# ATTron/astroz

Hardware: AMD Instinct MI355X
Metric: propagations/sec, 13,478 sats x 1,440 times, at 1/2/4/8 MI355X (higher is better)
Workload: dtype f64

## Files before the change

astroz_amd/csrc/astroz_hip.hip:

```cpp
#include "../../include/astroz_hip.h"

#include <hip/hip_runtime.h>
#include <dlfcn.h>
#include <rccl/rccl.h>

#include <algorithm>
#include <atomic>
#include <cmath>
#include <condition_variable>
#include <deque>
#include <map>
#include <cstdio>
#include <cstdlib>
#include <cstring>
#include <mutex>
#include <new>
#include <memory>
#include <string>
#include <thread>
#include <type_traits>
#include <vector>

#include "kernels.h"
#include "passes_kernel.h"
// ... 729 lines not shown
    if (c->d_times.ensure(n_times) != AZ_OK) return AZ_ERR_HIP;
    HIP_TRY(hipMemcpyAsync(c->d_times.p, times, sizeof(double) * n_times, hipMemcpyHostToDevice, st));
    c->have_offsets = offsets != nullptr;
    if (offsets) {
        if (c->d_offsets.ensure(c->n) != AZ_OK) return AZ_ERR_HIP;
        HIP_TRY(hipMemcpyAsync(c->d_offsets.p, offsets, sizeof(double) * c->n, hipMemcpyHostToDevice, st));
    }
    c->have_mask = mask != nullptr;
    if (mask) {
        if (c->d_mask.ensure(c->n) != AZ_OK) return AZ_ERR_HIP;
        HIP_TRY(hipMemcpyAsync(c->d_mask.p, mask, c->n, hipMemcpyHostToDevice, st));
    }
    if (mode != AZ_OUT_TEME) {
        if (c->d_sin.ensure(n_times) != AZ_OK || c->d_cos.ensure(n_times) != AZ_OK) return AZ_ERR_HIP;
        hipLaunchKernelGGL(k_gmst, dim3((unsigned)((n_times + 255) / 256)), dim3(256), 0, st, c->d_times.p,
                           (unsigned)n_times, reference_jd, c->d_sin.p, c->d_cos.p);
        HIP_TRY(hipGetLastError());
    }
    c->cached_n_times = (unsigned)n_times;
    c->cached_mode = mode;
    c->seeds_valid = false;
    drop_graphs(c);
    for (auto &pl : c->plan) pl.valid = false;
    c->last_plan = -1;
    c->uniform_step = 0.0;
    c->delta_max = 0.0;
    c->delta_wide = false;
    c->grid_t0 = n_times ? times[0] : 0.0;
    if (n_times >= 2) {
        double t0 = times[0], step = (times[n_times - 1] - t0) / (double)(n_times - 1);
        double tmax = std::max(std::fabs(t0), std::fabs(times[n_times - 1]));
        const double tol = 4.0 * 2.220446049250313e-16 * std::max(tmax, std::fabs(step));
        bool uni = std::isfinite(step) && step != 0.0;
        double dmax = 0.0;
        for (size_t i = 1; uni && i < n_times; ++i) {
            dmax = std::max(dmax, std::fabs(times[i] - std::fma((double)i, step, t0)));
            uni = dmax <= AZ_DELTA_MAX;
        }
        if (uni && dmax > tol) {
            c->h_delta.assign(n_times + AZ_DELTA_SEG, 0.0f);
            for (size_t i = 0; i < n_times; ++i) c->h_delta[i] = (float)(times[i] - std::fma((double)i, step, t0));
            if (c->d_delta.ensure(c->h_delta.size()) != AZ_OK) return AZ_ERR_HIP;
            HIP_TRY(hipMemcpyAsync(c->d_delta.p, c->h_delta.data(), sizeof(float) * c->h_delta.size(), hipMemcpyHostToDevice, st));
            c->h_delta64.assign(n_times + AZ_DELTA_SEG, 0.0);
            for (size_t i = 0; i < n_times; ++i) c->h_delta64[i] = times[i] - std::fma((double)i, step, t0);
            if (c->d_delta64.ensure(c->h_delta64.size()) != AZ_OK) return AZ_ERR_HIP;
            HIP_TRY(hipMemcpyAsync(c->d_delta64.p, c->h_delta64.data(), sizeof(double) * c->h_delta64.size(), hipMemcpyHostToDevice, st));
            c->delta_max = dmax * (1.0 + 1e-6) + 1e-12;
        }
        if (!uni && n_times >= 64) {
            const double nn = (double)n_times, im = 0.5 * (nn - 1.0);
            double tm = 0.0;
            for (size_t i = 0; i < n_times; ++i) tm += times[i];
            tm /= nn;
            double sxy = 0.0, sxx = 0.0;
            for (size_t i = 0; i < n_times; ++i) {
                sxy += ((double)i - im) * (times[i] - tm);
                sxx += ((double)i - im) * ((double)i - im);
            }
            step = sxy / sxx;
            t0 = tm - step * im;
            bool ok = std::isfinite(step) && std::isfinite(t0) && step != 0.0;
            dmax = 0.0;
            for (size_t i = 0; ok && i < n_times; ++i) {
                dmax = std::max(dmax, std::fabs(times[i] - std::fma((double)i, step, t0)));
                ok = dmax <= AZ_DELTA_WIDE_MAX;
            }
            if (ok && dmax <= 0.5 * std::fabs(step)) {
                c->h_delta64.assign(n_times + AZ_DELTA_SEG, 0.0);
                for (size_t i = 0; i < n_times; ++i) c->h_delta64[i] = times[i] - std::fma((double)i, step, t0);
                if (c->d_delta64.ensure(c->h_delta64.size()) != AZ_OK) return AZ_ERR_HIP;
                HIP_TRY(hipMemcpyAsync(c->d_delta64.p, c->h_delta64.data(), sizeof(double) * c->h_delta64.size(), hipMemcpyHostToDevice, st));
                c->delta_max = dmax * (1.0 + 1e-6) + 1e-12;
                c->delta_wide = true;
                c->grid_t0 = t0;
                uni = true;
            }
        }
        if (uni) {
            if (c->d_inc.ensure((size_t)2 * AZ_INC_NUM * c->n_pad) != AZ_OK) return AZ_ERR_HIP;
            hipLaunchKernelGGL(k_prep_inc, dim3((unsigned)((c->n + 255) / 256)), dim3(256), 0, st, c->d_el.p, c->n, c->n_pad,
                               step, c->d_inc.p);
            HIP_TRY(hipGetLastError());
            if (c->d_fast_rec.ensure((size_t)FR_NUM * c->n_pad) != AZ_OK) return AZ_ERR_HIP;
            hipLaunchKernelGGL(k_prep_rec, dim3((unsigned)((c->n + 255) / 256)), dim3(256), 0, st, c->d_el.p, c->d_flags.p, c->n, c->n_pad,
                               c->d_inc.p, c->d_fast_rec.p);
            HIP_TRY(hipGetLastError());
            c->uniform_step = step;
        }
    }
    try {
        c->h_times.assign(times, times + n_times);
        if (offsets) c->h_offsets.assign(offsets, offsets + c->n);
        if (mask) c->h_mask.assign(mask, mask + c->n);
        c->staged_ref_jd = reference_jd;
        c->staged_stream = st;
        c->staged_valid = true;
    } catch (const std::bad_alloc &) {
        c->staged_valid = false;
    }
    return AZ_OK;
}

int32_t prepare_deep(azh_constellation *c, PropArgs &d, hipStream_t st, bool rows, bool beside_bulk = false)
{
    const unsigned n_times = d.n_times;
    d.list = c->d_list.p + (rows ? c->off_deep_cat : c->n_sgp4);
    d.n_list = c->n_sdp4;
    d.tile = auto_tile(c->n_sdp4, n_times, c->tile_sdp4, 8);
    d.tile_forced = c->tile_sdp4 ? c->tile_sdp4 : (rows && beside_bulk && c->n_sgp4 >= 4u * c->n_sdp4 ? rows_tile(c->n_sgp4, n_times, c->tile_sgp4) : 0u);
    const unsigned seed_tile = rows ? 64u : d.tile;
    const unsigned n_tiles = (n_times + seed_tile - 1) / seed_tile;
    if (!c->seeds_valid || c->seeds_tile != seed_tile || c->seeds_rows != rows) {
        if (c->capturing) return AZ_RC_EAGER;
        drop_graphs(c);
        if (c->d_seeds.ensure((size_t)n_tiles * 3 * c->n_sdp4) != AZ_OK) return AZ_ERR_HIP;
        if (c->d_node_cache.p == nullptr) {
            if (c->d_node_cache.ensure(3 * c->n_pad) != AZ_OK) return AZ_ERR_HIP;
            HIP_TRY(hipMemsetAsync(c->d_node_cache.p, 0, sizeof(double) * 3 * c->n_pad, st));
        }
        hipLaunchKernelGGL(k_deep_seed, dim3((c->n_sdp4 + 63) / 64), dim3(64), 0, st, c->d_el.p, c->d_flags.p, c->n_pad,
                           d.list, c->n_sdp4, d.times, n_times, d.offsets, seed_tile, c->d_seeds.p, rows ? 1 : 0, c->d_node_cache.p);
        HIP_TRY(hipGetLastError());
        c->seeds_valid = true;
        c->seeds_tile = seed_tile;
        c->seeds_rows = rows;
    }
    d.seeds = c->d_seeds.p;
    return AZ_OK;
}

int32_t ensure_plan(azh_constellation *c, PropArgs &a, const FastShape &shape, hipStream_t st)
{
    azh_constellation::FastPlan &pl = c->plan[shape.kind];
    const unsigned n_list = a.n_list;
    const unsigned n_seg = (a.n_times + std::min(shape.tile_c, shape.tile_e) - 1) / std::min(shape.tile_c, shape.tile_e);
    if (!pl.valid || pl.tile_c != shape.tile_c || pl.tile_e != shape.tile_e || pl.n_list != n_list || pl.mixed32 != shape.mixed32) {
        if (c->capturing) return AZ_RC_EAGER;
        drop_graphs(c);
        const size_t items = (size_t)n_list * n_seg + ((size_t)a.n_times + 63) / 64 * (c->n_sgp4 - c->n_circ);
        if (pl.redo.cap < 4 + 3 * items || pl.win.cap < (size_t)n_list * n_seg * AZ_PLAN_NUM) HIP_TRY(hipStreamSynchronize(st));
        if (pl.redo.ensure(4 + 3 * items) != AZ_OK || pl.win.ensure((size_t)n_list * n_seg * AZ_PLAN_NUM) != AZ_OK ||
            pl.flag.ensure((size_t)n_list * n_seg) != AZ_OK)
            return AZ_ERR_HIP;
        HIP_TRY(hipMemsetAsync(pl.redo.p, 0, 4 * sizeof(unsigned), st));
        HIP_TRY(hipMemsetAsync(pl.flag.p, 0, (size_t)n_list * n_seg, st));
        PlanArgs q{};
        q.el = a.el; q.flags = a.flags; q.n_pad = a.n_pad; q.list = a.list; q.n_list = n_list; q.n_circ = a.n_circ;
        q.n_times = a.n_times; q.tile_c = shape.tile_c; q.tile_e = shape.tile_e; q.by_flags = shape.kind == 2 ? 1u : 0u;
        q.times = a.times; q.offsets = a.offsets; q.inc = a.inc; q.step = a.uniform_step; q.dt_mult = shape.kind == 1 ? 128.0 : 64.0;
        q.delta_max = (a.delta || a.delta64) ? a.delta_max : 0.0;
        q.grid_t0 = a.grid_t0;
        q.f32_mixed = shape.mixed32 ? 1u : 0u;
        q.win = pl.win.p; q.flag = pl.flag.p;
        q.redo_static = pl.redo.p + 2; q.redo_c0 = pl.redo.p; q.redo_c1 = pl.redo.p + 1; q.redo_items = pl.redo.p + 4;
        q.g = a.g;
        hipLaunchKernelGGL(k_plan_windows, dim3((n_list + 255) / 256, n_seg), dim3(256), 0, st, q);
        hipLaunchKernelGGL(k_plan_arm, dim3(1), dim3(64), 0, st, q.redo_static, q.redo_c0, q.redo_c1);
        HIP_TRY(hipGetLastError());
        pl.valid = true;
        pl.tile_c = shape.tile_c; pl.tile_e = shape.tile_e; pl.n_list = n_list; pl.n_seg = n_seg; pl.parity = 0; pl.mixed32 = shape.mixed32;
    }
    c->last_plan = (int)shape.kind;
    a.plan_win = pl.win.p;
    a.plan_flag = pl.flag.p;
    a.plan_stride = n_list;
    a.redo_static = pl.redo.p + 2;
    a.redo_count = pl.redo.p + pl.parity;
    a.redo_next = pl.redo.p + (pl.parity ^ 1u);
// ... 2921 lines not shown
```

astroz_amd/csrc/fast_step.h:

```cpp
#pragma once
#include <type_traits>

#include "propagate_device.h"

#define AZ_FASTK_COLD(X)                                                                                     \
    X(cc1) X(d2) X(d3) X(d4) X(nl2) X(nl3) X(nl4) X(nl5) X(eta) X(omgcof) X(xmcof) X(xd) X(bc4) X(bc5) X(ecb) X(sab)
#define AZ_FASTK_HOT(X)                                                                                      \
    X(aycof) X(xlcof) X(xnodcf) X(sinio) X(cosio) X(k_mrt) X(k_c2u) X(k_su) X(k_node) X(k_inc) X(x1mth2) X(k_rv) \
    X(sdA) X(cdA) X(sdW) X(cdW) X(tc) X(sdU) X(cdU) X(tmid) X(nodedot) X(sOc) X(cOc)
enum FastCold {
#define X(n) FC_##n,
    AZ_FASTK_COLD(X)
#undef X
    FC_NUM
};
#define AZ_FASTK_DELTA(X) X(mdot) X(argpdot) X(udot)
enum FastColdX {
    FCX_first_ = FC_NUM - 1,
#define X(n) FCX_##n,
    AZ_FASTK_DELTA(X)
#undef X
    FCX_NUM
};
#define AZ_DELTA_MAX 4.0e-6
// ... 86 lines not shown
AZ_DEVICE void az_fast_udot(FastK &k) { k.udot_ = fma(2.0 * k.nl2_, k.tc_, k.mdot_ + k.argpdot_); }

template <class K>
AZ_DEVICE void az_fast_window(const double *__restrict__ el, size_t n_pad, size_t i, double t_a, double t_b, double dt, K &k)
{
#define L(f) el[(size_t)F_##f * n_pad + i]
    const double kappa = L(no_unkozai) * L(t2cof);
    const double tmax = fmax(fabs(t_a), fabs(t_b));
    k.tmid_ = 0.5 * (t_a + t_b);
    az_sincos(fma(k.nodedot_, k.tmid_, L(nodeo)), k.sOc_, k.cOc_);
    if (!az_any(fabs(kappa) * tmax * tmax > 0.05)) {
        k.tc_ = 0.0;
        k.sdU_ = fma(k.sdA_, k.cdW_, k.cdA_ * k.sdW_);
        k.cdU_ = fma(k.cdA_, k.cdW_, -(k.sdA_ * k.sdW_));
    } else {
        k.tc_ = 0.5 * (t_a + t_b);
        az_sincos((L(mdot) + L(argpdot) + 2.0 * kappa * k.tc_) * dt, k.sdU_, k.cdU_);
    }
    if constexpr (std::is_same<K, FastK>::value) az_fast_udot(k);
#undef L
}

#define AZ_FASTK_HOT_REC(X)                                                                                  \
    X(aycof) X(xlcof) X(xnodcf) X(sinio) X(cosio) X(k_mrt) X(k_c2u) X(k_su) X(k_node) X(k_inc) X(x1mth2) X(k_rv) \
    X(sdA) X(cdA) X(sdW) X(cdW) X(nodedot)
enum FastRec {
    FR_COLD0 = 0,
    FR_HOT0 = FCX_NUM,
#define X(n) FR_##n,
    FR_first_hot_ = FR_HOT0 - 1,
    AZ_FASTK_HOT_REC(X)
#undef X
    FR_mo, FR_mdot, FR_argpo, FR_argpdot,
    FR_USED,
    FR_NUM = (FR_USED + 7) & ~7
};
AZ_DEVICE void az_fast_rec_store(const double *__restrict__ el, size_t n_pad, size_t i, const FastK &k, double *__restrict__ rec)
{
#define X(n) rec[FC_##n] = k.n##_;
    AZ_FASTK_COLD(X)
#undef X
    rec[FCX_mdot] = k.mdot_; rec[FCX_argpdot] = k.argpdot_; rec[FCX_udot] = k.mdot_ + k.argpdot_;
#define X(n) rec[FR_##n] = k.n##_;
    AZ_FASTK_HOT_REC(X)
#undef X
#define L(f) el[(size_t)F_##f * n_pad + i]
    rec[FR_mo] = L(mo); rec[FR_mdot] = L(mdot); rec[FR_argpo] = L(argpo); rec[FR_argpdot] = L(argpdot);
#undef L
    for (int j = FR_USED; j < FR_NUM; ++j) rec[j] = 0.0;
}
template <class K, class P = const double *__restrict__>
AZ_DEVICE void az_fast_rec_hot(P rec, K &k)
{
#define X(n) k.n##_ = rec[FR_##n];
    AZ_FASTK_HOT_REC(X)
#undef X
}
template <class M>
AZ_DEVICE void az_seed_fast_rec(const double *__restrict__ rec, double kappa, double t, double tc, FastCarry &st, const M &m)
{
    az_sincos_m(fma(rec[FR_mdot], t, rec[FR_mo]), st.sA, st.cA, m);
    az_sincos_m(fma(rec[FR_argpdot], t, rec[FR_argpo]), st.sW, st.cW, m);
    if (!az_any(tc != 0.0)) {
        st.sU = fma(st.sA, st.cW, st.cA * st.sW);
        st.cU = fma(st.cA, st.cW, -(st.sA * st.sW));
    } else {
        az_sincos_m(fma(rec[FR_mdot] + rec[FR_argpdot] + 2.0 * kappa * tc, t, rec[FR_mo] + rec[FR_argpo] - kappa * tc * tc), st.sU, st.cU, m);
    }
}

AZ_DEVICE void az_seed_fast(const double *__restrict__ el, size_t n_pad, size_t i, double t, double tc, FastCarry &st)
{
#define L(f) el[(size_t)F_##f * n_pad + i]
    az_sincos(fma(L(mdot), t, L(mo)), st.sA, st.cA);
    az_sincos(fma(L(argpdot), t, L(argpo)), st.sW, st.cW);
    if (!az_any(tc != 0.0)) {
        st.sU = fma(st.sA, st.cW, st.cA * st.sW);
        st.cU = fma(st.cA, st.cW, -(st.sA * st.sW));
    } else {
        const double kappa = L(no_unkozai) * L(t2cof);
        az_sincos(fma(L(mdot) + L(argpdot) + 2.0 * kappa * tc, t, L(mo) + L(argpo) - kappa * tc * tc), st.sU, st.cU);
    }
#undef L
}

AZ_DEVICE void az_rot_apply2(double &s, double &c, double p, double q)
{
    const double ns = fma(c, p, fma(s, q, s));
    c = fma(-s, p, fma(c, q, c));
    s = ns;
}
enum RotCoef { RC_n6, RC_p24, RC_p120, RC_n720, RC_n5040, RC_p40320, RC_p362880, RC_n3628800, RC_p8,
               RC_n11f, RC_p12f, RC_p13f, RC_n14f, RC_n15f, RC_p16f, RC_NUM };
#define AZ_RC_VALUES                                                                                                      \
    {-1.0 / 6.0, 1.0 / 24.0, 1.0 / 120.0, -1.0 / 720.0, -1.0 / 5040.0, 1.0 / 40320.0, 1.0 / 362880.0, -1.0 / 3628800.0, 0.125,     \
     -1.0 / 39916800.0, 1.0 / 479001600.0, 1.0 / 6227020800.0, -1.0 / 87178291200.0, -1.0 / 1307674368000.0,                   \
     1.0 / 20922789888000.0}
struct RotCoefLit {
    AZ_MEMBER double operator()(int k) const
    {
        constexpr double v[RC_NUM] = AZ_RC_VALUES;
        return v[k];
    }
};
struct RotCoefLds {
    const double *p;
    AZ_MEMBER double operator()(int k) const { return p[k]; }
};
template <class W>
AZ_DEVICE void az_rotcoef_store(W write)
{
    const RotCoefLit lit;
#pragma unroll
    for (int k = 0; k < RC_NUM; ++k) write(k, lit(k));
}

template <class RC>
AZ_DEVICE void az_rotate_tiny2(double &s, double &c, double d, const RC &k)
{
    const double d2 = d * d;
    const double q = -0.5 * d2;
    const double p = fma(d2 * k(RC_n6), d, d);
    az_rot_apply2(s, c, p, q);
}
template <class RC>
AZ_DEVICE void az_fpq_small(double d, const RC &k, double &p, double &q)
{
    const double d2 = d * d;
    q = d2 * fma(d2, fma(d2, k(RC_n720), k(RC_p24)), -0.5);
    p = d * fma(d2, fma(d2, k(RC_p120), k(RC_n6)), 1.0);
}

#define AZ_ROT_16TH 0.0625
template <class RC>
AZ_DEVICE void az_pq_16th(double d, const RC &k, double &p, double &q)
{
    const double d2 = d * d;
    q = d2 * fma(d2, fma(d2, fma(d2, k(RC_p40320), k(RC_n720)), k(RC_p24)), -0.5);
    p = d * fma(d2, fma(d2, fma(d2, k(RC_n5040), k(RC_p120)), k(RC_n6)), 1.0);
}

template <class RC>
AZ_DEVICE void az_pq_large(double d, const RC &k, double &p, double &q)
{
    const double d2 = d * d;
    q = fma(d2, k(RC_p16f), k(RC_n14f));
    q = fma(d2, q, k(RC_p12f));
    q = fma(d2, q, k(RC_n3628800));
    q = fma(d2, q, k(RC_p40320));
    q = fma(d2, q, k(RC_n720));
    q = fma(d2, q, k(RC_p24));
    q = d2 * fma(d2, q, -0.5);
    p = fma(d2, k(RC_n15f), k(RC_p13f));
    p = fma(d2, p, k(RC_n11f));
    p = fma(d2, p, k(RC_p362880));
    p = fma(d2, p, k(RC_n5040));
    p = fma(d2, p, k(RC_p120));
    p = fma(d2, p, k(RC_n6));
    p = d * fma(d2, p, 1.0);
}

template <class RC>
AZ_DEVICE void az_pq_med(double d, const RC &k, double &p, double &q)
{
    const double d2 = d * d;
    q = fma(d2, k(RC_n3628800), k(RC_p40320));
// ... 300 lines not shown
```

astroz_amd/csrc/kernels.h:

```cpp
#pragma once
#include <hip/hip_runtime.h>

#include <type_traits>

#include "init_device.h"
#include "propagate_device.h"
#include "fast_step.h"
#include "fast_step_f32.h"

#ifndef AZ_BLOCK
#define AZ_BLOCK 256
#endif
#ifndef AZ_PROP_FAST
#define AZ_PROP_FAST 1
#endif
#ifndef AZ_MIN_WAVES
#define AZ_MIN_WAVES 1
#endif
#ifndef AZ_ROWS_WAVES
#define AZ_ROWS_WAVES 3
#endif
#ifndef AZ_DEEP_WAVES
#define AZ_DEEP_WAVES 2
#endif
#define AZ_RESEED 256
#ifndef AZ_SM_CHUNK
#define AZ_SM_CHUNK 4
#endif

struct PropArgs {
    const double *el;
    const unsigned *flags;
    size_t n_pad;
    const unsigned *list;
    unsigned n_list;
    const double *times;
    unsigned n_times;
    const double *offsets;
    double *pos, *vel;
    const double *sin_g, *cos_g;
    const unsigned char *mask;
    unsigned char *err;
    size_t stride_sats;
    unsigned tile;
    unsigned tile_e, screen_nseg;
    unsigned tile_forced;
    const double *seeds;
    int mode;
    int f32;
    int tm_rows;
    int rows_compact;
    unsigned ecc_row0;
    const double *screen_target;
    union {
        double *part_d2;
        const AzObserver *obs;
    };
    unsigned *part_t;
    double uniform_step;
    int grid_exact_uniform;
    const float *delta;
    double delta_max;
    const double *delta64;
    int delta_wide;
    double grid_t0;
    const double *inc;
    const double *fast_rec;
    unsigned row_lo, row_hi;
    unsigned slot_lo, slot_hi;
    unsigned win_circ_lo, win_circ_hi, win_ecc_lo, win_ecc_hi;
    int arith32;
    unsigned n_circ;
    unsigned redo_slot0;
    unsigned *redo_count;
    unsigned *redo_next;
    unsigned *redo_items;
    const unsigned *rowmap;
    const double *tmp_pos, *tmp_vel;
    unsigned n_rows;
    const double *plan_win;
    const unsigned char *plan_flag;
    unsigned plan_stride;
    const unsigned *redo_static;
    AzGrav g;
};
enum { AZ_ROW_NEAR = 0, AZ_ROW_COPY = 1, AZ_ROW_ZERO = 2 };
enum { AZ_PLAN_sOc, AZ_PLAN_cOc, AZ_PLAN_sdU, AZ_PLAN_cdU, AZ_PLAN_s1U, AZ_PLAN_c1U, AZ_PLAN_NUM };
#define AZ_PLAN_OK 1u
#define AZ_PLAN_TC 2u
#define AZ_PLAN_TIER_SHIFT 2
#define AZ_PLAN_TIER_MASK 1u
#define AZ_PLAN_ETIER_MASK 3u
#ifndef AZ_ROWS_ETIERS
#define AZ_ROWS_ETIERS 1
#endif
#define AZ_PLAN_ECC 16u
#define AZ_PLAN_SET 32u

template <class T>
__device__ __forceinline__ void az_put3(T *o, const double r[3])
{
    o[0] = (T)r[0];
    o[1] = (T)r[1];
    o[2] = (T)r[2];
}
typedef double az_d2s __attribute__((ext_vector_type(2), aligned(8)));
typedef float az_f3s __attribute__((ext_vector_type(3), aligned(4)));
#ifndef AZ_ROWS_NT
#define AZ_ROWS_NT 1
#endif
__device__ __forceinline__ void az_put3_stream(double *o, const double r[3])
{
#if AZ_ROWS_NT
    const az_d2s a = {r[0], r[1]};
    __builtin_nontemporal_store(a, reinterpret_cast<az_d2s *>(o));
    __builtin_nontemporal_store(r[2], o + 2);
#else
    az_put3(o, r);
#endif
}
__device__ __forceinline__ void az_put3_stream(float *o, const double r[3])
{
#if AZ_ROWS_NT
    const az_f3s a = {(float)r[0], (float)r[1], (float)r[2]};
    __builtin_nontemporal_store(a, reinterpret_cast<az_f3s *>(o));
#else
    az_put3(o, r);
#endif
}

__device__ __forceinline__ void az_epilogue(double r[3], double v[3], int mode, bool vel, const double *sin_g,
                                            const double *cos_g, unsigned i)
{
    if (mode != 0) {
        const double sg = sin_g[i], cg = cos_g[i];
        az_to_ecef(r, sg, cg);
        if (vel) az_to_ecef(v, sg, cg);
        if (mode == 2) az_ecef_to_geodetic(r);
    }
}
template <bool VEL>
__device__ __forceinline__ void az_epilogue_topo(double r[3], double v[3], const PropArgs &p, unsigned i)
{
    const double sg = p.sin_g[i], cg = p.cos_g[i];
    az_to_ecef(r, sg, cg);
    if (VEL) az_to_ecef(v, sg, cg);
    az_topocentric<VEL>(r, v, *p.obs);
}

#define AZ_TM_ROW 256
#define AZ_SM_ROW (AZ_SM_CHUNK * 3 + 1)

typedef double az_d2 __attribute__((ext_vector_type(2)));

#if defined(AZ_STORE_POLICY) && AZ_STORE_POLICY == 1
#define AZ_ST1(ptr, val) __builtin_nontemporal_store((val), (ptr))
#define AZ_ST2(ptr, val) __builtin_nontemporal_store((val), (ptr))
#else
#define AZ_ST1(ptr, val) (*(ptr) = (val))
#define AZ_ST2(ptr, val) (*(ptr) = (val))
#endif

__device__ __forceinline__ double az_readlane_f64(double x, unsigned lane_uniform)
{
    const int lo = __builtin_amdgcn_readlane(__double2loint(x), (int)lane_uniform);
    const int hi = __builtin_amdgcn_readlane(__double2hiint(x), (int)lane_uniform);
    return __hiloint2double(hi, lo);
}

__device__ __forceinline__ void az_wave_lds_fence()
// ... 308 lines not shown
    }
    if (node_cache && in_range && e.irez != 0 && have_near) {
        node_cache[s] = near.atime;
        node_cache[n_pad + s] = near.xli;
        node_cache[2 * n_pad + s] = near.xni;
    }
}

#ifndef AZ_ONE_SEG
#define AZ_ONE_SEG 1024
#endif
#define AZ_ONE_LISTS 64u
#define AZ_ONE_HEAD (32u * AZ_ONE_LISTS)
template <bool ITEMS = false>
__global__ void __launch_bounds__(64) k_one_satellite(const double *__restrict__ el, const unsigned *__restrict__ flags,
                                                            size_t n_pad, unsigned sat, const double *__restrict__ tsince,
                                                            unsigned n, double *pos, double *vel,
                                                            unsigned char *err, int interleaved, AzGrav g,
                                                            const double *__restrict__ offsets, int nan_on_error,
                                                            const unsigned *__restrict__ items = nullptr, unsigned list_cap = 0)
{
    const unsigned sub = ITEMS ? (blockIdx.x % AZ_ONE_LISTS) : 0u;
    const unsigned n_work = ITEMS ? items[32u * sub] * (AZ_ONE_SEG / 64u) : 1u;
#pragma unroll 1
    for (unsigned w = ITEMS ? blockIdx.x / AZ_ONE_LISTS : 0u; w < n_work; w += ITEMS ? gridDim.x / AZ_ONE_LISTS : 1u) {
    const unsigned i = ITEMS ? items[AZ_ONE_HEAD + sub * list_cap + w / (AZ_ONE_SEG / 64u)] * AZ_ONE_SEG + (w % (AZ_ONE_SEG / 64u)) * 64u + threadIdx.x
                             : blockIdx.x * 64 + threadIdx.x;
    if (ITEMS && i - threadIdx.x >= n) continue;
    const double t = tsince[i < n ? i : n - 1] + (offsets ? offsets[sat] : 0.0);
    const unsigned fl = flags[sat];
    double r[3], v[3];
    int rc = AZ_FLAG_ERR(fl);
    if (rc == 0) {
        if (fl & AZ_FLAG_DEEP) {
            Sdp4Lane e;
            Sdp4Carry c;
            __shared__ double cold_deep[D_NUM * 64];
            double *cold = cold_deep + threadIdx.x;
            az_load_sdp4(el, n_pad, sat, fl, e, ColdLds{cold});
            c.atime = 0.0;
            c.xli = e(H_xlamo);
            c.xni = e(H_no_unkozai);
            rc = az_sdp4_step<true>(e, ColdLds{cold}, g, az_rotk(), t, c, r, v);
        } else {
            Sgp4Lane e;
            Sgp4Carry c;
            ColdRegs cold;
            az_load_sgp4(el, n_pad, sat, fl, e, cold);
            c.t_prev = 0.0;
            az_sgp4_step<true>(e, cold, el, n_pad, sat, g, az_rotk(), t, true, c, r, v);
        }
    }
    if (rc != 0) {
        r[0] = r[1] = r[2] = nan_on_error ? __builtin_nan("") : 0.0;
        v[0] = v[1] = v[2] = 0.0;
    }
    if (i < n) {
        if (interleaved) {
            double *o = pos + (size_t)i * 6;
            o[0] = r[0]; o[1] = r[1]; o[2] = r[2]; o[3] = v[0]; o[4] = v[1]; o[5] = v[2];
        } else {
            pos[(size_t)i * 3] = r[0]; pos[(size_t)i * 3 + 1] = r[1]; pos[(size_t)i * 3 + 2] = r[2];
            if (vel) { vel[(size_t)i * 3] = v[0]; vel[(size_t)i * 3 + 1] = v[1]; vel[(size_t)i * 3 + 2] = v[2]; }
        }
        if (err) err[i] = (unsigned char)rc;
    }
    }
}

struct PlanArgs {
    const double *el;
    const unsigned *flags;
    size_t n_pad;
    const unsigned *list;
    unsigned n_list, n_circ, n_times, tile_c, tile_e, by_flags;
    unsigned f32_mixed;
    const double *times, *offsets, *inc;
    double step, dt_mult, delta_max, grid_t0;
    double *win;
    unsigned char *flag;
    unsigned *redo_static, *redo_c0, *redo_c1, *redo_items;
    AzGrav g;
};
__global__ void __launch_bounds__(256) k_plan_windows(PlanArgs a)
{
    const unsigned slot = blockIdx.x * 256 + threadIdx.x;
    const unsigned seg = blockIdx.y;
    if (slot >= a.n_list) return;
    const unsigned s = a.list[slot];
    const unsigned fl = a.flags[s];
    const bool ecc = a.by_flags ? AZ_FLAG_ECLASS(fl) != 0 : slot >= a.n_circ;
    const unsigned tile = ecc ? a.tile_e : a.tile_c;
    const unsigned t_lo = seg * tile;
    if (t_lo >= a.n_times) return;
    const unsigned t_hi = min(t_lo + tile, a.n_times);
    const double t_first = a.grid_t0 + (a.offsets ? a.offsets[s] : 0.0);
    const double w_a = fma((double)t_lo, a.step, t_first), w_b = fma((double)(t_hi - 1), a.step, t_first);
    FastK k0, k1;
    az_load_fast(a.el, a.n_pad, s, fl, a.inc, 0, k0);
    const double dt_mult = ecc ? 64.0 : a.dt_mult;
    if (dt_mult == 128.0) az_double_increments(k0);
    az_fast_window(a.el, a.n_pad, s, w_a, w_b, dt_mult * a.step, k0);
    az_load_fast(a.el, a.n_pad, s, fl, a.inc, 1, k1);
    az_fast_window(a.el, a.n_pad, s, w_a, w_b, a.step, k1);
    int tier = ecc ? az_fast_window_tier<true>(k0, a.g, w_a, w_b, a.delta_max) : az_fast_window_tier<false>(k0, a.g, w_a, w_b, a.delta_max);
    if (ecc && (AZ_ROWS_ETIERS == 0 || (AZ_ROWS_ETIERS == 2 && tier == AZ_ETIER_E2))) tier = min(tier, (int)AZ_TIER_GENERAL);
    bool ok = tier >= 0;
    if (!ecc && AZ_FLAG_ECLASS(fl) != 0) ok = false;
    if (!ecc && a.f32_mixed && !az_fast32p_window_ok(k0, w_a, w_b)) ok = false;
    const size_t at = (size_t)seg * a.n_list + slot;
    double *w = a.win + at * AZ_PLAN_NUM;
    w[AZ_PLAN_sOc] = k0.sOc_; w[AZ_PLAN_cOc] = k0.cOc_; w[AZ_PLAN_sdU] = k0.sdU_; w[AZ_PLAN_cdU] = k0.cdU_;
    w[AZ_PLAN_s1U] = k1.sdU_; w[AZ_PLAN_c1U] = k1.cdU_;
    a.flag[at] = (unsigned char)((ok ? AZ_PLAN_OK | ((unsigned)tier << AZ_PLAN_TIER_SHIFT) : 0u) | (k0.tc_ != 0.0 ? AZ_PLAN_TC : 0u) |
                                 (ecc ? AZ_PLAN_ECC : 0u) | AZ_PLAN_SET);
    if (!ok) {
        const unsigned k = atomicAdd(a.redo_static, 1u);
        a.redo_items[3 * (size_t)k + 0] = slot;
        a.redo_items[3 * (size_t)k + 1] = t_lo;
        a.redo_items[3 * (size_t)k + 2] = t_hi;
    }
}
__global__ void k_plan_arm(unsigned *redo_static, unsigned *c0, unsigned *c1)
{
    if (threadIdx.x == 0 && blockIdx.x == 0) *c0 = *c1 = *redo_static;
}
template <class K>
__device__ __forceinline__ bool az_plan_window(const PropArgs &p, unsigned seg, unsigned slot, double w_a, double w_b, K &k0, unsigned *tier = nullptr)
{
    const size_t at = (size_t)seg * p.plan_stride + slot;
    const double *w = p.plan_win + at * AZ_PLAN_NUM;
    const unsigned f = p.plan_flag[at];
    k0.tmid_ = 0.5 * (w_a + w_b);
    k0.tc_ = (f & AZ_PLAN_TC) ? k0.tmid_ : 0.0;
    k0.sOc_ = w[AZ_PLAN_sOc]; k0.cOc_ = w[AZ_PLAN_cOc]; k0.sdU_ = w[AZ_PLAN_sdU]; k0.cdU_ = w[AZ_PLAN_cdU];
    if (tier) *tier = (f >> AZ_PLAN_TIER_SHIFT) & ((f & AZ_PLAN_ECC) ? AZ_PLAN_ETIER_MASK : AZ_PLAN_TIER_MASK);
    return (f & AZ_PLAN_OK) != 0;
}

AZ_DEVICE double az_uniform(double x)
{
#ifdef AZ_HOST_EMUL
    return x;
#else
    return __hiloint2double(__builtin_amdgcn_readfirstlane(__double2hiint(x)),
                            __builtin_amdgcn_readfirstlane(__double2loint(x)));
#endif
}
AZ_DEVICE float az_uniform32(float x)
{
#ifdef AZ_HOST_EMUL
    return x;
#else
    return __int_as_float(__builtin_amdgcn_readfirstlane(__float_as_int(x)));
#endif
}
__device__ __forceinline__ const double *az_opaque_lds(const double *p)
{
    typedef __attribute__((address_space(3))) const double lds_cdouble;
    lds_cdouble *q = (lds_cdouble *)p;
    asm volatile("" : "+v"(q));
    return (const double *)q;
}
struct ColdBroadcast;
struct ColdBroadcast {
    double *p;
    const double *m = nullptr;
    __device__ __forceinline__ double operator()(int k) const { return p[k]; }
    __device__ __forceinline__ void set(int k, double v) const { p[k] = v; }
    __device__ __forceinline__ double mc(int k) const { return m[k]; }
    __device__ __forceinline__ ColdBroadcast fresh() const;
};
struct ColdBroadcastLit {
    double *p;
    __device__ __forceinline__ double operator()(int k) const { return p[k]; }
    __device__ __forceinline__ void set(int k, double v) const { p[k] = v; }
    __device__ __forceinline__ double mc(int k) const { return az_mc_literal(k); }
    __device__ __forceinline__ const ColdBroadcastLit &fresh() const { return *this; }
};
__device__ const double az_mc_table[MC_NUM] = AZ_MC_VALUES;
__device__ const double az_rc_table[RC_NUM] = AZ_RC_VALUES;
#define AZ_SC_NUM (MC_C5 + 1)
#define AZ_FAST_TABLE ((FCX_NUM + RC_NUM + AZ_SC_NUM + 1) & ~1)
struct McLds {
    const double *p;
    __device__ __forceinline__ double mc(int k) const { return p[k]; }
};
__device__ __forceinline__ void az_fill_fast_table(double *table, const double *__restrict__ rec, unsigned lane)
{
    static_assert(FCX_NUM + RC_NUM + AZ_SC_NUM <= 64, "one lane per table entry");
    const double *src = lane < FCX_NUM ? rec + lane
                        : lane < FCX_NUM + RC_NUM ? az_rc_table + (lane - FCX_NUM) : az_mc_table + (lane - (FCX_NUM + RC_NUM));
    if (lane < FCX_NUM + RC_NUM + AZ_SC_NUM) table[lane] = *src;
}
__device__ __forceinline__ ColdBroadcast ColdBroadcast::fresh() const { return ColdBroadcast{p, az_opaque_lds(m)}; }
#ifndef AZ_ROWSF_WAVES
// ... 125 lines not shown
    const bool ecc = AZ_FLAG_ECLASS(fl) != 0;
    bool ok = AZ_FLAG_ERR(fl) == 0 && !(fl & AZ_FLAG_DEEP) && cnt >= 128u;
    double t0 = 0.0, step = 0.0;
    FastK k;
    if (ok) {
        t0 = az_uniform(tsince[lo]) + off;
        step = ((az_uniform(tsince[lo + cnt - 1]) + off) - t0) / (double)(cnt - 1u);
        bool far = false;
#pragma unroll 4
        for (unsigned j = lane; j < (unsigned)AZ_ONE_SEG; j += 64u) {
            const unsigned jj = min(j, cnt - 1u);
            const double d = (tsince[lo + jj] + off) - fma((double)jj, step, t0);
            dl_lds[j] = (float)d;
            far |= !(fabs(d) <= AZ_DELTA_MAX);
        }
        ok = !az_any(far) && step != 0.0 && fabs(step) * (double)cnt <= 3000.0;
    }
    if (ok) {
#define L(f) el[(size_t)F_##f * n_pad + sat]
        double sdA, cdA, sdW, cdW;
        az_sincos(L(mdot) * (64.0 * step), sdA, cdA);
        az_sincos(L(argpdot) * (64.0 * step), sdW, cdW);
#undef L
        az_load_fast_with(el, n_pad, sat, fl, sdA, cdA, sdW, cdW, k);
        const double w_a = t0, w_b = fma((double)(cnt - 1u), step, t0);
        az_fast_window(el, n_pad, sat, w_a, w_b, 64.0 * step, k);
        ok = ecc ? az_fast_window_ok<true>(k, g, w_a, w_b, AZ_DELTA_MAX) : az_fast_window_ok<false>(k, g, w_a, w_b, AZ_DELTA_MAX);
    }
    if (ok) {
        FastCarry fc;
        az_seed_fast(el, n_pad, sat, fma((double)lane - 64.0, step, t0), k.tc_, fc);
        double *prow = pos + (size_t)lo * 3, *vrow = VEL ? vel + (size_t)lo * 3 : nullptr;
        const bool staged = ((reinterpret_cast<size_t>(prow) | (VEL ? reinterpret_cast<size_t>(vrow) : 0)) & 15u) == 0;
        const AzRowSink sink = az_row_sink(prow, vrow, cnt);
        az_wave_lds_fence();
#pragma unroll 1
        for (unsigned base = 0; base < cnt; base += 64u) {
            const unsigned i = base + lane;
            const bool live = i < cnt;
            const double dl = (double)dl_lds[i];
            const double t = fma((double)i, step, t0) + dl;
            double r[3], v[3];
            const bool bad = ecc ? az_sgp4_fast_step<VEL, true, 1>(k, g, RotCoefLit(), t, fc, r, v, dl)
                                 : az_sgp4_fast_step<VEL, false, 1>(k, g, RotCoefLit(), t, fc, r, v, dl);
            if (az_any(bad && live)) {
                ok = false;
                break;
            }
            az_rows_store<VEL>(staged, base + 64u <= cnt, live, lane, rows_stage, prow, vrow, base, r, v, sink);
            if (err && live) err[lo + i] = 0;
        }
    }
    if (!ok && lane == 0) {
        const unsigned sub = seg % AZ_ONE_LISTS;
        items[AZ_ONE_HEAD + sub * list_cap + atomicAdd(items + 32u * sub, 1u)] = seg;
    }
}

#define AZ_FRAME_SEG 256
template <bool VEL, int FRAME, int SINK, bool ECC, int DELTA = 0>
__global__ void __launch_bounds__(64, FRAME >= 2 ? 4 : (ECC ? AZ_ROWSF_ECC_WAVES : (FRAME == 1 || DELTA == 2 ? 5 : AZ_ROWSF_WAVES))) k_rows_fast(PropArgs p)
{
    typedef typename std::conditional<SINK == AZ_SINK_F32, float, double>::type out_t;
    const unsigned lane = threadIdx.x;
    const unsigned row = az_list_slot(p);
    [[maybe_unused]] const AzObserver obs = FRAME == 3 ? *p.obs : AzObserver{};
    if (row >= az_list_end(p)) return;
    const unsigned s = p.list[row];
    if (SINK != AZ_SINK_SCREEN && ((p.mask != nullptr && p.mask[s] == 0) || s < p.row_lo || s >= p.row_hi)) return;
    const unsigned t_lo = blockIdx.y * p.tile;
    if (t_lo >= p.n_times) return;
    const unsigned t_hi = min(t_lo + p.tile, p.n_times);
    unsigned base = t_lo;
    bool window_ok;
    unsigned tier = AZ_TIER_GENERAL;
    double best_d2 = __builtin_inf();
    unsigned best_t = 0xffffffffu;
    {
        __shared__ __attribute__((aligned(16))) double cold_lds[AZ_FAST_TABLE];
        __shared__ __attribute__((aligned(16))) out_t rows_stage[AZ_ROWS_LDS_STORE ? 2 * 64 * 3 : 4];
        const double off = az_uniform(p.offsets ? p.offsets[s] : 0.0);
        const double *__restrict__ rec = p.fast_rec + (size_t)s * FR_NUM;
        az_fill_fast_table(cold_lds, rec, lane);
        const size_t out_row = p.rows_compact ? (size_t)p.ecc_row0 + row : (size_t)s;
        out_t *prow = SINK == AZ_SINK_SCREEN ? nullptr : reinterpret_cast<out_t *>(p.pos) + out_row * p.n_times * 3;
        out_t *vrow = VEL ? reinterpret_cast<out_t *>(p.vel) + out_row * p.n_times * 3 : nullptr;
        const bool staged = AZ_ROWS_LDS_STORE && SINK != AZ_SINK_SCREEN &&
                            (((reinterpret_cast<size_t>(prow) | (VEL ? reinterpret_cast<size_t>(vrow) : 0)) & 15u) == 0);
        FastKBcast k;
        {
            const double w_a = fma((double)t_lo, p.uniform_step, p.grid_t0 + off), w_b = fma((double)(t_hi - 1), p.uniform_step, p.grid_t0 + off);
            window_ok = az_plan_window(p, blockIdx.y, row + p.redo_slot0, w_a, w_b, k, &tier);
            if (!window_ok) return;
            az_fast_rec_hot(rec, k);
            az_wave_lds_fence();
            if (DELTA && k.tc_ != 0.0 && lane == 0) cold_lds[FCX_udot] = fma(2.0 * rec[FC_nl2], k.tc_, rec[FCX_udot]);
        }
        typedef typename std::conditional<DELTA == 2, double, float>::type dl_t;
        __shared__ dl_t dl_lds[DELTA ? AZ_DELTA_SEG : 1];
        if (DELTA) {
            const dl_t *src = DELTA == 2 ? reinterpret_cast<const dl_t *>(p.delta64) : reinterpret_cast<const dl_t *>(p.delta);
#pragma unroll
            for (unsigned j = lane; j < AZ_DELTA_SEG; j += 64) dl_lds[j] = src[t_lo + j];
        }
        az_wave_lds_fence();
        const double step = p.uniform_step;
        const double t_first = p.grid_t0 + off;
        FastCarry fc;
        az_seed_fast_rec(rec, rec[FC_nl2], fma((double)(t_lo + lane) - 64.0, step, t_first), k.tc_, fc,
                         McLds{cold_lds + FCX_NUM + RC_NUM});
        __shared__ double gst_lds[FRAME ? 2 * AZ_FRAME_SEG : 2];
        if (FRAME) {
#pragma unroll
            for (unsigned j = lane; j < AZ_FRAME_SEG; j += 64) {
                const unsigned jj = min(t_lo + j, p.n_times - 1);
                gst_lds[2 * j] = p.sin_g[jj];
                gst_lds[2 * j + 1] = p.cos_g[jj];
            }
            az_wave_lds_fence();
        }
        AzRowSink sink{};
        if constexpr (SINK != AZ_SINK_SCREEN) sink = az_row_sink(prow, vrow, p.n_times);
        auto run = [&](auto tier_c, const unsigned t_end) __attribute__((always_inline)) {
        constexpr int TIER = decltype(tier_c)::value;
#pragma unroll 1
        for (; window_ok && base < t_end; base += 64) {
            const unsigned i = base + lane;
            const bool live = i < t_hi;
            double t = fma((double)i, step, t_first), dl = 0.0;
            if (DELTA) {
                dl = (double)dl_lds[i - t_lo];
                t += dl;
            }
            const double *cold_now = az_opaque_lds(cold_lds);
            k.cold = cold_now;
            const RotCoefLds rk{cold_now + FCX_NUM};
            double r[3], v[3];
#if defined(AZ_ABLATE) && AZ_ABLATE == 2
            r[0] = t; r[1] = t + 1.0; r[2] = t + 2.0; v[0] = t + 3.0; v[1] = t + 4.0; v[2] = t + 5.0;
#else
            const bool bad = az_sgp4_fast_step<VEL, ECC, DELTA, TIER>(k, p.g, rk, t, fc, r, v, dl);
            if (az_any(bad && live)) break;
#endif
            if (SINK == AZ_SINK_SCREEN) {
                const double *q = p.screen_target + (size_t)(live ? i : t_hi - 1) * 3;
                const double dx = q[0] - r[0], dy = q[1] - r[1], dz = q[2] - r[2];
                const double d2 = fma(dx, dx, fma(dy, dy, dz * dz));
                if (live && d2 < best_d2) {
                    best_d2 = d2;
                    best_t = i;
                }
                continue;
            }
            if (FRAME) {
                if (((base - t_lo) & (AZ_FRAME_SEG - 1u)) == 0u && base != t_lo) {
                    az_wave_lds_fence();
#pragma unroll
                    for (unsigned j = lane; j < AZ_FRAME_SEG; j += 64) {
                        const unsigned jn = min(base + j, p.n_times - 1);
                        gst_lds[2 * j] = p.sin_g[jn];
                        gst_lds[2 * j + 1] = p.cos_g[jn];
                    }
                    az_wave_lds_fence();
                }
                const unsigned jj = (i - t_lo) & (AZ_FRAME_SEG - 1u);
                const double sg = gst_lds[2 * jj], cg = gst_lds[2 * jj + 1];
                az_to_ecef(r, sg, cg);
                if (VEL) az_to_ecef(v, sg, cg);
                if (FRAME == 2) az_ecef_to_geodetic(r);
                if (FRAME == 3) az_topocentric<VEL>(r, v, obs);
            }
#if defined(AZ_ABLATE) && AZ_ABLATE == 1
            if (!(live && (r[0] + r[1] + r[2] + (VEL ? v[0] + v[1] + v[2] : 0.0)) == 1.2345e300)) continue;
#endif
            az_rows_store<VEL>(staged, base + 64 <= t_hi, live, lane, rows_stage, prow, vrow, base, r, v, sink);
        }
        };
        if constexpr (AZ_ROWS_TIERS && !ECC && FRAME == 0) run(std::integral_constant<int, AZ_TIER_EPS>(), tier == AZ_TIER_EPS ? t_hi : t_lo);
        if constexpr (AZ_ROWS_ETIERS && ECC && FRAME == 0 && DELTA != 2) {
            run(std::integral_constant<int, AZ_ETIER_E1>(), tier == AZ_ETIER_E1 ? t_hi : t_lo);
            if constexpr (AZ_ROWS_ETIERS == 1) run(std::integral_constant<int, AZ_ETIER_E2>(), tier == AZ_ETIER_E2 ? t_hi : t_lo);
        }
        run(std::integral_constant<int, AZ_TIER_GENERAL>(), t_hi);
    }
    if (SINK == AZ_SINK_SCREEN) {
        az_wave_argmin(best_d2, best_t);
        if (lane == 0) {
            p.part_d2[(size_t)blockIdx.y * p.plan_stride + row + p.redo_slot0] = best_d2;
            p.part_t[(size_t)blockIdx.y * p.plan_stride + row + p.redo_slot0] = best_t;
        }
    }
// ... 767 lines not shown
    const unsigned *occ = a.occupied + (size_t)k * words;
    for (int dx = -1; dx <= 1; ++dx)
        for (int dy = -1; dy <= 1; ++dy)
            for (int dz = -1; dz <= 1; ++dz) {
                const int nx = c[0] + dx, ny = c[1] + dy, nz = c[2] + dz;
                const unsigned h = az_cell_hash(nx, ny, nz) & a.table_mask;
                const unsigned word = staged ? bits[h >> 5] : occ[h >> 5];
                if (!((word >> (h & 31u)) & 1u)) continue;
                unsigned idx = head[h];
                while (idx != 0xffffffffu) {
                    const unsigned other = idx;
                    idx = next[other];
                    if (other <= s) continue;
                    double q[3];
                    int oc[3];
                    az_cell_of(a, other, t, q, oc);
                    if (oc[0] != nx || oc[1] != ny || oc[2] != nz) continue;
                    const double ex = r[0] - q[0], ey = r[1] - q[1], ez = r[2] - q[2];
                    if (ex * ex + ey * ey + ez * ez < a.thr2) {
                        const unsigned long long w = atomicAdd(a.count, 1ull);
                        if (w < a.max_results) {
                            a.out_pairs[2 * w] = s;
                            a.out_pairs[2 * w + 1] = other;
                            a.out_t[w] = t;
                        }
                    }
                }
            }
}

__global__ void k_fill_bad(const unsigned *list, unsigned n_list, const unsigned *flags, unsigned n_times,
                           double *pos, double *vel, unsigned char *err, const unsigned char *mask, int layout,
                           size_t stride_sats, int f32, unsigned row_lo, unsigned row_hi)
{
    const unsigned i = blockIdx.x * blockDim.x + threadIdx.x;
    const unsigned li = blockIdx.y;
    if (i >= n_times || li >= n_list) return;
    const unsigned s = list[li];
    if ((mask && !mask[s]) || s < row_lo || s >= row_hi) return;
    const size_t ob = (layout == 0) ? ((size_t)s * n_times + i) * 3 : ((size_t)i * stride_sats + s) * 3;
    if (f32) {
        float *p32 = reinterpret_cast<float *>(pos), *v32 = reinterpret_cast<float *>(vel);
        p32[ob] = p32[ob + 1] = p32[ob + 2] = 0.0f;
        if (vel) v32[ob] = v32[ob + 1] = v32[ob + 2] = 0.0f;
    } else {
        pos[ob] = pos[ob + 1] = pos[ob + 2] = 0.0;
        if (vel) vel[ob] = vel[ob + 1] = vel[ob + 2] = 0.0;
    }
    if (err) err[(size_t)s * n_times + i] = (unsigned char)AZ_FLAG_ERR(flags[s]);
}

__global__ void k_gmst(const double *times, unsigned n, double reference_jd, double *sin_g, double *cos_g)
{
    const unsigned i = blockIdx.x * blockDim.x + threadIdx.x;
    if (i >= n) return;
    const double d = (reference_jd + times[i] / 1440.0) - 2451545.0;
    const double tc = d / 36525.0;
    double gm = 280.46061837 + 360.98564736629 * d + 0.000387933 * tc * tc - tc * tc * tc / 38710000.0;
    gm = fmod(gm, 360.0);
    if (gm < 0) gm += 360.0;
    gm *= AZ_PI / 180.0;
    sin_g[i] = sin(gm);
    cos_g[i] = cos(gm);
}

__global__ void __launch_bounds__(256) k_prep_inc(const double *el, size_t n, size_t n_pad, double step, double *inc)
{
    const size_t s = (size_t)blockIdx.x * 256 + threadIdx.x;
    if (s >= n) return;
    const double rate[2] = {el[(size_t)F_mdot * n_pad + s], el[(size_t)F_argpdot * n_pad + s]};
#pragma unroll
    for (int which = 0; which < 2; ++which) {
        const double dt = which == 0 ? 64.0 * step : step;
#pragma unroll
        for (int a = 0; a < 2; ++a) {
            double sn, cs;
            az_sincos(rate[a] * dt, sn, cs);
            inc[(size_t)(AZ_INC_NUM * which + 2 * a) * n_pad + s] = sn;
            inc[(size_t)(AZ_INC_NUM * which + 2 * a + 1) * n_pad + s] = cs;
        }
    }
}

__global__ void __launch_bounds__(256) k_prep_rec(const double *el, const unsigned *flags, size_t n, size_t n_pad, const double *inc, double *rec)
{
    const size_t s = (size_t)blockIdx.x * 256 + threadIdx.x;
    if (s >= n) return;
    FastK k;
    az_load_fast(el, n_pad, s, flags[s], inc, 0, k);
    az_fast_rec_store(el, n_pad, s, k, rec + s * FR_NUM);
}

__global__ void k_coords(int op, const double *in, double *out)
{
    if (threadIdx.x != 0 || blockIdx.x != 0) return;
    if (op == 0) {
        const double d = in[0] - 2451545.0;
        const double tc = d / 36525.0;
        double gm = 280.46061837 + 360.98564736629 * d + 0.000387933 * tc * tc - tc * tc * tc / 38710000.0;
        gm = fmod(gm, 360.0);
        if (gm < 0) gm += 360.0;
        out[0] = gm * (AZ_PI / 180.0);
        out[1] = out[2] = 0.0;
    } else if (op == 1) {
        double r[3] = {in[0], in[1], in[2]};
        az_to_ecef(r, sin(in[3]), cos(in[3]));
        out[0] = r[0]; out[1] = r[1]; out[2] = r[2];
    } else if (op == 2) {
        double r[3] = {in[0], in[1], in[2]};
        az_ecef_to_geodetic(r);
        out[0] = r[0] * (180.0 / AZ_PI); out[1] = r[1] * (180.0 / AZ_PI); out[2] = r[2];
    } else if (op == 3) {
        const double mu = in[0], r = in[1], a = in[2];
        out[0] = sqrt(a != 0.0 ? mu * (2.0 / r - 1.0 / a) : mu / r);
        out[1] = 2.0 * AZ_PI * sqrt(a * a * a / mu);
        out[2] = sqrt(2.0 * mu / r);
    } else {
        const double mu = in[0], r1 = in[1], r2 = in[2];
        const double sma = 0.5 * (r1 + r2), v1c = sqrt(mu / r1), v2c = sqrt(mu / r2);
        const double dv1 = v1c * sqrt(2.0 * r2 / (r1 + r2)) - v1c, dv2 = v2c - v2c * sqrt(2.0 * r1 / (r1 + r2));
        out[0] = sma; out[1] = dv1; out[2] = dv2; out[3] = fabs(dv1) + fabs(dv2); out[4] = AZ_PI * sqrt(sma * sma * sma / mu);
    }
}

__global__ void __launch_bounds__(64) k_math_kat(const double *x, unsigned n, double *out)
{
    const unsigned i = blockIdx.x * 64 + threadIdx.x;
    const double v = x[i < n ? i : n - 1];
    double sn, cs;
    az_sincos(v, sn, cs);
    const double rc = az_rcp(v), rs = az_rsqrt(fabs(v));
    double s0 = 0.6684330296514408, c0 = 0.7437723340317224;
    az_rotate(s0, c0, v, az_rotk());
    if (i < n) {
        out[i] = sn; out[n + i] = cs; out[2 * (size_t)n + i] = v * rc; out[3 * (size_t)n + i] = fabs(v) * rs * rs;
        out[4 * (size_t)n + i] = s0; out[5 * (size_t)n + i] = c0;
    }
}

__global__ void __launch_bounds__(64) k_init(const double *raw, size_t n, size_t n_pad, AzGrav g, double *el,
                                                   unsigned *flags)
{
    const size_t s = (size_t)blockIdx.x * 64 + threadIdx.x;
    if (s >= n) return;
    double in[AZ_NUM_RAW];
#pragma unroll
    for (int k = 0; k < AZ_NUM_RAW; ++k) in[k] = raw[(size_t)k * n_pad + s];
    flags[s] = az_init_satellite(in, g, el, n_pad, s);
}
```

Measured before the change: 97.45 billion.

## Seed per-lane carries from precomputed angle tables instead of per-lane sincos

Adds a per-satellite table of sin/cos of j*rate*step and 8j*rate*step for mean anomaly and argument of perigee, built in a new prep kernel. The plan kernel stores the base-angle sin/cos per window. The row kernel then seeds each lane's rotation carry with two complex multiplies instead of computing fresh sincos calls. The plan kernel also drops the tc (t^2 drag) term per satellite when its contribution over the window is small, so more windows can take the table path. This costs extra memory, a new prep launch, an LDS stage, and some accuracy risk from compounded rotations and the tc threshold.

```diff
diff --git a/astroz_amd/csrc/astroz_hip.hip b/astroz_amd/csrc/astroz_hip.hip
--- a/astroz_amd/csrc/astroz_hip.hip
+++ b/astroz_amd/csrc/astroz_hip.hip
@@ -835,9 +835,12 @@
             hipLaunchKernelGGL(k_prep_inc, dim3((unsigned)((c->n + 255) / 256)), dim3(256), 0, st, c->d_el.p, c->n, c->n_pad,
                                step, c->d_inc.p);
             HIP_TRY(hipGetLastError());
-            if (c->d_fast_rec.ensure((size_t)FR_NUM * c->n_pad) != AZ_OK) return AZ_ERR_HIP;
+            if (c->d_fast_rec.ensure((size_t)(FR_NUM + AZ_SEEDTAB_NUM) * c->n_pad) != AZ_OK) return AZ_ERR_HIP;
             hipLaunchKernelGGL(k_prep_rec, dim3((unsigned)((c->n + 255) / 256)), dim3(256), 0, st, c->d_el.p, c->d_flags.p, c->n, c->n_pad,
                                c->d_inc.p, c->d_fast_rec.p);
+            HIP_TRY(hipGetLastError());
+            hipLaunchKernelGGL(k_prep_seed_tab, dim3((unsigned)((c->n * 32 + 255) / 256)), dim3(256), 0, st, c->d_el.p, c->n, c->n_pad,
+                               step, c->d_fast_rec.p + (size_t)FR_NUM * c->n_pad);
             HIP_TRY(hipGetLastError());
             c->uniform_step = step;
         }
diff --git a/astroz_amd/csrc/fast_step.h b/astroz_amd/csrc/fast_step.h
--- a/astroz_amd/csrc/fast_step.h
+++ b/astroz_amd/csrc/fast_step.h
@@ -192,6 +192,51 @@
         az_sincos(fma(L(mdot) + L(argpdot) + 2.0 * kappa * tc, t, L(mo) + L(argpo) - kappa * tc * tc), st.sU, st.cU);
     }
 #undef L
+}
+
+#ifndef AZ_SEED_TABLES
+#define AZ_SEED_TABLES 1
+#endif
+enum { AZ_SEEDTAB_FINE = 0, AZ_SEEDTAB_COARSE = 16, AZ_SEEDTAB_ANGLE = 32, AZ_SEEDTAB_NUM = 64 };
+AZ_DEVICE void az_seed_table_entry(double rate, double step, int m, double &s, double &c)
+{
+    const double d = rate * step, dlo = fma(rate, step, -d);
+    const double fm = (double)m, a = fm * d;
+    const double e = fma(fm, dlo, fma(fm, d, -a));
+    double sa, ca;
+    az_sincos(a, sa, ca);
+    s = fma(ca, e, sa);
+    c = fma(-sa, e, ca);
+}
+AZ_DEVICE void az_seed_table_store(double mdot, double argpdot, double step, double *__restrict__ tab)
+{
+    for (int e = 0; e < AZ_SEEDTAB_NUM / 2; ++e) {
+        const int j = e & 7, coarse = (e >> 3) & 1;
+        az_seed_table_entry((e >> 4) ? argpdot : mdot, step, coarse ? 8 * j : j, tab[2 * e], tab[2 * e + 1]);
+    }
+}
+AZ_DEVICE void az_seed_base(double mo, double mdot, double argpo, double argpdot, double t_base, double base[4])
+{
+    az_sincos(fma(mdot, t_base, mo), base[0], base[1]);
+    az_sincos(fma(argpdot, t_base, argpo), base[2], base[3]);
+}
+AZ_DEVICE void az_seed_fast_tab(const double *__restrict__ tab, unsigned lane, double sA0, double cA0, double sW0, double cW0, FastCarry &st)
+{
+    const double *f = tab + AZ_SEEDTAB_FINE + 2u * (lane & 7u), *g = tab + AZ_SEEDTAB_COARSE + 2u * (lane >> 3);
+    {
+        const double sg = g[0], cg = g[1], sf = f[0], cf = f[1];
+        const double s1 = fma(sA0, cg, cA0 * sg), c1 = fma(cA0, cg, -(sA0 * sg));
+        st.sA = fma(s1, cf, c1 * sf);
+        st.cA = fma(c1, cf, -(s1 * sf));
+    }
+    {
+        const double sg = g[AZ_SEEDTAB_ANGLE], cg = g[AZ_SEEDTAB_ANGLE + 1], sf = f[AZ_SEEDTAB_ANGLE], cf = f[AZ_SEEDTAB_ANGLE + 1];
+        const double s1 = fma(sW0, cg, cW0 * sg), c1 = fma(cW0, cg, -(sW0 * sg));
+        st.sW = fma(s1, cf, c1 * sf);
+        st.cW = fma(c1, cf, -(s1 * sf));
+    }
+    st.sU = fma(st.sA, st.cW, st.cA * st.sW);
+    st.cU = fma(st.cA, st.cW, -(st.sA * st.sW));
 }
 
 AZ_DEVICE void az_rot_apply2(double &s, double &c, double p, double q)
diff --git a/astroz_amd/csrc/kernels.h b/astroz_amd/csrc/kernels.h
--- a/astroz_amd/csrc/kernels.h
+++ b/astroz_amd/csrc/kernels.h
@@ -85,7 +85,7 @@
     AzGrav g;
 };
 enum { AZ_ROW_NEAR = 0, AZ_ROW_COPY = 1, AZ_ROW_ZERO = 2 };
-enum { AZ_PLAN_sOc, AZ_PLAN_cOc, AZ_PLAN_sdU, AZ_PLAN_cdU, AZ_PLAN_s1U, AZ_PLAN_c1U, AZ_PLAN_NUM };
+enum { AZ_PLAN_sOc, AZ_PLAN_cOc, AZ_PLAN_sdU, AZ_PLAN_cdU, AZ_PLAN_s1U, AZ_PLAN_c1U, AZ_PLAN_sA0, AZ_PLAN_cA0, AZ_PLAN_sW0, AZ_PLAN_cW0, AZ_PLAN_NUM };
 #define AZ_PLAN_OK 1u
 #define AZ_PLAN_TC 2u
 #define AZ_PLAN_TIER_SHIFT 2
@@ -560,6 +560,20 @@
     unsigned *redo_static, *redo_c0, *redo_c1, *redo_items;
     AzGrav g;
 };
+#ifndef AZ_PLAN_TC_VOTE
+#define AZ_PLAN_TC_VOTE 0
+#endif
+AZ_DEVICE void az_fast_window_own(const double *__restrict__ el, size_t n_pad, size_t i, double t_a, double t_b, FastK &k)
+{
+    const double kappa = el[(size_t)F_no_unkozai * n_pad + i] * el[(size_t)F_t2cof * n_pad + i];
+    const double tmax = fmax(fabs(t_a), fabs(t_b));
+    if (!(fabs(kappa) * tmax * tmax > 0.05) && k.tc_ != 0.0) {
+        k.tc_ = 0.0;
+        k.sdU_ = fma(k.sdA_, k.cdW_, k.cdA_ * k.sdW_);
+        k.cdU_ = fma(k.cdA_, k.cdW_, -(k.sdA_ * k.sdW_));
+        az_fast_udot(k);
+    }
+}
 __global__ void __launch_bounds__(256) k_plan_windows(PlanArgs a)
 {
     const unsigned slot = blockIdx.x * 256 + threadIdx.x;
@@ -581,6 +595,10 @@
     az_fast_window(a.el, a.n_pad, s, w_a, w_b, dt_mult * a.step, k0);
     az_load_fast(a.el, a.n_pad, s, fl, a.inc, 1, k1);
     az_fast_window(a.el, a.n_pad, s, w_a, w_b, a.step, k1);
+#if !AZ_PLAN_TC_VOTE
+    az_fast_window_own(a.el, a.n_pad, s, w_a, w_b, k0);
+    az_fast_window_own(a.el, a.n_pad, s, w_a, w_b, k1);
+#endif
     int tier = ecc ? az_fast_window_tier<true>(k0, a.g, w_a, w_b, a.delta_max) : az_fast_window_tier<false>(k0, a.g, w_a, w_b, a.delta_max);
     if (ecc && (AZ_ROWS_ETIERS == 0 || (AZ_ROWS_ETIERS == 2 && tier == AZ_ETIER_E2))) tier = min(tier, (int)AZ_TIER_GENERAL);
     bool ok = tier >= 0;
@@ -590,6 +608,13 @@
     double *w = a.win + at * AZ_PLAN_NUM;
     w[AZ_PLAN_sOc] = k0.sOc_; w[AZ_PLAN_cOc] = k0.cOc_; w[AZ_PLAN_sdU] = k0.sdU_; w[AZ_PLAN_cdU] = k0.cdU_;
     w[AZ_PLAN_s1U] = k1.sdU_; w[AZ_PLAN_c1U] = k1.cdU_;
+    {
+#define L(f) a.el[(size_t)F_##f * a.n_pad + s]
+        double base[4];
+        az_seed_base(L(mo), L(mdot), L(argpo), L(argpdot), fma((double)t_lo - 64.0, a.step, t_first), base);
+#undef L
+        w[AZ_PLAN_sA0] = base[0]; w[AZ_PLAN_cA0] = base[1]; w[AZ_PLAN_sW0] = base[2]; w[AZ_PLAN_cW0] = base[3];
+    }
     a.flag[at] = (unsigned char)((ok ? AZ_PLAN_OK | ((unsigned)tier << AZ_PLAN_TIER_SHIFT) : 0u) | (k0.tc_ != 0.0 ? AZ_PLAN_TC : 0u) |
                                  (ecc ? AZ_PLAN_ECC : 0u) | AZ_PLAN_SET);
     if (!ok) {
@@ -881,6 +906,10 @@
         const double off = az_uniform(p.offsets ? p.offsets[s] : 0.0);
         const double *__restrict__ rec = p.fast_rec + (size_t)s * FR_NUM;
         az_fill_fast_table(cold_lds, rec, lane);
+#if AZ_SEED_TABLES
+        __shared__ __attribute__((aligned(16))) double seed_lds[AZ_SEEDTAB_NUM];
+        seed_lds[lane] = p.fast_rec[(size_t)FR_NUM * p.n_pad + (size_t)s * AZ_SEEDTAB_NUM + lane];
+#endif
         const size_t out_row = p.rows_compact ? (size_t)p.ecc_row0 + row : (size_t)s;
         out_t *prow = SINK == AZ_SINK_SCREEN ? nullptr : reinterpret_cast<out_t *>(p.pos) + out_row * p.n_times * 3;
         out_t *vrow = VEL ? reinterpret_cast<out_t *>(p.vel) + out_row * p.n_times * 3 : nullptr;
@@ -906,6 +935,12 @@
         const double step = p.uniform_step;
         const double t_first = p.grid_t0 + off;
         FastCarry fc;
+#if AZ_SEED_TABLES
+        if (k.tc_ == 0.0) {
+            const double *w = p.plan_win + ((size_t)blockIdx.y * p.plan_stride + row + p.redo_slot0) * AZ_PLAN_NUM;
+            az_seed_fast_tab(seed_lds, lane, w[AZ_PLAN_sA0], w[AZ_PLAN_cA0], w[AZ_PLAN_sW0], w[AZ_PLAN_cW0], fc);
+        } else
+#endif
         az_seed_fast_rec(rec, rec[FC_nl2], fma((double)(t_lo + lane) - 64.0, step, t_first), k.tc_, fc,
                          McLds{cold_lds + FCX_NUM + RC_NUM});
         __shared__ double gst_lds[FRAME ? 2 * AZ_FRAME_SEG : 2];
@@ -1839,6 +1874,15 @@
     }
 }
 
+__global__ void __launch_bounds__(256) k_prep_seed_tab(const double *el, size_t n, size_t n_pad, double step, double *tab)
+{
+    const size_t idx = (size_t)blockIdx.x * 256 + threadIdx.x, s = idx >> 5;
+    if (s >= n) return;
+    const int e = (int)(idx & 31u), j = e & 7;
+    az_seed_table_entry(el[(size_t)((e >> 4) ? F_argpdot : F_mdot) * n_pad + s], step, ((e >> 3) & 1) ? 8 * j : j,
+                        tab[s * AZ_SEEDTAB_NUM + 2 * e], tab[s * AZ_SEEDTAB_NUM + 2 * e + 1]);
+}
+
 __global__ void __launch_bounds__(256) k_prep_rec(const double *el, const unsigned *flags, size_t n, size_t n_pad, const double *inc, double *rec)
 {
     const size_t s = (size_t)blockIdx.x * 256 + threadIdx.x;
```

After: 98.54 billion, median of 6. 1.1% higher.
